# tesseract-robotics/trajopt

Measured on NVIDIA H100. Metric: converged trajectories/sec (7-DOF x 30 wp, batch 1024), higher is better.
Workload: dtype f64

## Files before the change

### trajopt_b200/csrc/kernels.h

```cpp
#pragma once
#include "device_types.cuh"

namespace tb200 {
struct EvalExtra;
struct SolveCtl;
using SolveKernelFn = void (*)(DevProblem, EvalExtra, SolveCtl);
using EvalKernelFn = void (*)(DevProblem, EvalExtra, int, const double*);
SolveKernelFn solve_kernel_for(int D, bool pair_rows, bool sing);
EvalKernelFn eval_kernel_for(int D, bool sing);
int eval_debug_prof(unsigned long long* out, int reset);
constexpr int kQpProfSlots = 32;
int qp_debug_prof(unsigned long long* out, int reset);
}
```

### trajopt_b200/csrc/qp_cta_kernel.cuh

```cuda
#pragma once
#include "device_types.cuh"
#include "joint_terms.cuh"

namespace tb200 {

#ifdef TB200_PROFILE
static __device__ unsigned long long g_prof[32];
#define PROF_T0() const long long prof_t0_ = clock64()
#define PROF_ADD(slot) do { if (q.tid == 0) atomicAdd(&g_prof[slot], (unsigned long long)(clock64() - prof_t0_)); } while (0)
#define PROF_COUNT(slot) do { if (q.tid == 0) atomicAdd(&g_prof[slot], 1ull); } while (0)
#define PROF_ADD2(slot, slot2) do { if (q.tid == 0) { const unsigned long long d_ = clock64() - prof_t0_; \
    atomicAdd(&g_prof[slot], d_); atomicAdd(&g_prof[slot2], d_); } } while (0)
#else
#define PROF_T0()
#define PROF_ADD(slot)
#define PROF_COUNT(slot)
#define PROF_ADD2(slot, slot2)
#endif
#if defined(TB200_PROFILE) && defined(TB200_PROFILE_CHECK)
#define PROF_CHK_T0() long long pc_ = clock64()
#define PROF_CHK(slot) do { const long long n_ = clock64(); if (q.tid == 0) atomicAdd(&g_prof[slot], (unsigned long long)(n_ - pc_)); pc_ = n_; } while (0)
#else
#define PROF_CHK_T0()
#define PROF_CHK(slot)
#endif

constexpr int kQpThreads = 256;
constexpr int kQpThreadsC = 256;
constexpr double kOsqpInf = 1e30;
constexpr double kMinScaling = 1e-4, kMaxScaling = 1e4;
constexpr double kVerifyTol = 1e-9;
constexpr int kVerifyRounds = 3;
constexpr double kRhoMin = 1e-6, kRhoMax = 1e6, kRhoTol = 1e-4, kRhoEqOverIneq = 1e3;
enum { QPS_UNSOLVED = 0, QPS_SOLVED = 1, QPS_SOLVED_INACC = 2, QPS_PINF = 3, QPS_PINF_INACC = 4, QPS_DINF = 5,
       QPS_DINF_INACC = 6, QPS_MAXITER = 7, QPS_NONCVX = 8 };

__device__ __forceinline__ double limit_scaling(double v) {
  v = v < kMinScaling ? 1.0 : v;
  return v > kMaxScaling ? kMaxScaling : v;
}

struct QpSmem {
  int SA, SLM, SU, beta, x, zb, yb, v1, w, qs, lbs, ubs, Dz, v2, Pb, tmp, red, colptr, colent, rints, rows, total, row_cap;
  int factor_smem, pband_smem;
  int pinv;
};

struct PinvPlan {
  int ok;
  int Ns, nS;
  int PR;
  int ZS, HO;
  int WS;
  int SS;
  int zo, wo, so;
  int total;
};
__host__ __device__ inline PinvPlan pinv_plan(int M, int nb) {
  PinvPlan pl;
  pl.Ns = M / 4;
  pl.nS = pl.Ns * nb;
  pl.PR = (M - pl.Ns) * nb;
  const int Np = M * nb, blk = nb * nb;
  pl.ok = (nb % 2 == 0) && nb <= 14 && pl.Ns <= 3 && pl.PR + 2 * pl.nS <= 256;
  pl.ZS = Np + ((4 - Np % 16) + 16) % 16;
  pl.HO = ((Np / 2 + 6) / 16) * 16 + 2;
  if (pl.HO > Np) pl.HO = Np;
  pl.WS = 2 * nb + 2;
  pl.SS = pl.nS + (pl.nS & 1);
  const int fA = (M * blk + 15) & ~15, fL = fA + 8, fU = (M * blk + 1) & ~1;
  const int zn = pl.nS * pl.ZS;
  pl.zo = 0;
  pl.wo = ((zn > fA + fL + fU ? zn : fA + fL + fU) + 15) & ~15;
  pl.so = pl.wo + ((pl.PR * pl.WS + 1) & ~1);
  pl.total = pl.so + pl.nS * pl.SS;
  return pl;
}
constexpr int kQpSmemBudget = 28800;
__host__ __device__ inline int qp_block_count(int N, int nb) { return (N + nb - 1) / nb; }
__host__ __device__ inline int qp_even(int v) { return (v + 1) & ~1; }
__host__ __device__ inline int qp_factor_doubles(int N, int nb) { return 3 * qp_even(qp_block_count(N, nb) * nb * nb); }
__host__ __device__ inline size_t qp_cta_global_doubles(int N, int nb) {
  const PinvPlan pl = pinv_plan(qp_block_count(N, nb), nb);
  return static_cast<size_t>(qp_factor_doubles(N, nb)) + static_cast<size_t>(pl.nS) * pl.ZS;
}
__host__ __device__ inline QpSmem qp_smem_layout(int N, int nb, int row_stride, int CN, int max_rows, bool factor_global) {
  const int M = qp_block_count(N, nb), Np = M * nb, blk = nb * nb;
  QpSmem s;
  int o = 0;
  s.beta = o; o += qp_even(Np);
  s.x = o;    o += qp_even(Np);
  s.zb = o;   o += qp_even(Np);
  s.yb = o;   o += qp_even(Np);
  s.v1 = o;   o += qp_even(Np);
  s.w = o;    o += qp_even(Np);
  s.qs = o;   o += qp_even(Np);
  s.lbs = o;  o += qp_even(Np);
  s.ubs = o;  o += qp_even(Np);
  s.Dz = o;   o += qp_even(Np);
  s.v2 = o;   o += qp_even(Np);
  s.tmp = o;  o += 2 * kQpThreadsC + 64 + 8;
  s.red = o;  o += 16 * 8;
  s.colptr = o; o += qp_even((Np + 2) / 2 + 1);
  const int fA = (M * blk + 15) & ~15, fL = fA + 8, fU = qp_even(M * blk);
  s.factor_smem = (!factor_global && o + fA + fL + fU <= kQpSmemBudget) ? 1 : 0;
  o = s.factor_smem ? ((o + 15) & ~15) : o;
  const int per_row2 = 2 * row_stride + CN + RI_NINTS;
  const PinvPlan pl = pinv_plan(M, nb);
  {
    const int region = qp_even(pl.total > fA + fL + fU ? pl.total : fA + fL + fU);
    const int o2 = o + region + qp_even(N * (nb + 1));
    const int cap2 = (o2 < kQpSmemBudget) ? 2 * (kQpSmemBudget - o2) / per_row2 - 1 : 0;
    s.pinv = (s.factor_smem && pl.ok && cap2 >= (max_rows < 64 ? max_rows : 64)) ? 1 : 0;
  }
  s.SA = o;   o += s.factor_smem ? fA : 0;
  s.SLM = o;  o += s.factor_smem ? fL : 0;
  s.SU = o;   o += s.factor_smem ? fU : 0;
  if (s.pinv && s.SA + pl.total > o) o = s.SA + qp_even(pl.total);
  s.pband_smem = (o + qp_even(N * (nb + 1)) <= kQpSmemBudget) ? 1 : 0;
  s.Pb = o;   o += s.pband_smem ? qp_even(N * (nb + 1)) : 0;
  int cap = (o < kQpSmemBudget) ? 2 * (kQpSmemBudget - o) / per_row2 - 1 : 0;
  cap = cap > max_rows ? max_rows : cap;
  cap = cap > 1023 ? 1023 : cap;
  cap = cap < 0 ? 0 : cap;
  s.row_cap = cap;
  s.colent = o; o += qp_even((cap * CN + 1) / 2);
  s.rints = o;  o += qp_even((cap * RI_NINTS + 1) / 2);
  s.rows = o;   o += cap * row_stride;
  s.total = o;
  return s;
}

enum RowF {
  R_C = 0, R_W,
  R_E, R_DA0, R_DA1, R_EA0, R_EA1,
  R_U0, R_U1, R_B0, R_B1, R_LO, R_UP, R_QA0, R_QA1, R_RHO,
  R_XA0, R_XA1, R_Z, R_Y, R_ZA0, R_ZA1, R_YA0, R_YA1,
  R_RA0, R_RA1, R_COEF, R_WR, R_G0, R_G1, R_DEN, R_WRR,
  R_IDEN, R_IWRR,
  R_DY, R_DYA0, R_DYA1, R_DXA0, R_DXA1,
  R_PW, R_PWA0, R_PWA1, R_PB, R_PY, R_PYA0, R_PYA1, R_PX0, R_PX1,
  R_MV,
  R_NF
};
__host__ __device__ inline int qp_row_stride(int CN) { return 3 * CN + R_NF; }

struct SmVec {
  int off;
  __device__ __forceinline__ double* ptr() const {
    extern __shared__ double sm[];
    return sm + off;
  }
  __device__ __forceinline__ double& operator[](int i) const { return ptr()[i]; }
  __device__ __forceinline__ operator double*() const { return ptr(); }
  __device__ __forceinline__ SmVec& operator=(double* p) {
    extern __shared__ double sm[];
    off = static_cast<int>(p - sm);
    return *this;
  }
};

struct QpCtx {
  int N, Np, nb, M, T, D, CN, RS, tid, nrows;
  double *SA, *SLM, *SU;
  SmVec beta, x, zb, yb, v1, w, qs, lbs, ubs, tmp, red, flag;
  int* colptr;
  SmVec Dz, v2;
  double* rows;
  double* soa;
  double* smbase;
  int rows_smem;
  int* rints;
  const int* colent;
  const double* Pband;
  const int* band_offs;
  int n_band;
  double* scratch;
  int pinv;
  PinvPlan pl;
  double* pi_g;
  double* z_stash;
  double c, cinv, rho, rho_eq, sigma, alpha;
  __device__ __forceinline__ double* R(int r) const { return rows + static_cast<size_t>(r) * RS; }
  __device__ __forceinline__ double* F(int r) const { return rows + static_cast<size_t>(r) * RS + 2 * CN; }
  __device__ __forceinline__ const int* I(int r) const { return rints + static_cast<size_t>(r) * RI_NINTS; }
};

__device__ __forceinline__ double warp_max_norm(double v) {
  v = (v != v) ? 0.0 : v;
  const unsigned hi = static_cast<unsigned>(__double2hiint(v)) & 0x7fffffffu, lo = static_cast<unsigned>(__double2loint(v));
  const unsigned mh = __reduce_max_sync(0xffffffffu, hi);
  const unsigned ml = __reduce_max_sync(0xffffffffu, hi == mh ? lo : 0u);
  return __hiloint2double(static_cast<int>(mh), static_cast<int>(ml));
}
template <int NQ, unsigned SUM_MASK>
__device__ __forceinline__ void block_reduce(const QpCtx& q, double (&vals)[NQ]) {
  static_assert(NQ <= 16, "red area too small");
  extern __shared__ double sm[];
  double* const red = sm + (q.red - q.smbase);
  const int lane = q.tid & 31, wid = q.tid >> 5;
  __syncwarp();
#pragma unroll
  for (int k = 0; k < NQ; ++k) {
    double v = vals[k];
    if ((SUM_MASK >> k) & 1u) {
#pragma unroll
      for (int off = 16; off > 0; off >>= 1) v += __shfl_xor_sync(0xffffffffu, v, off);
    } else {
      v = warp_max_norm(v);
    }
    vals[k] = v;
  }
  if (lane == 0) {
#pragma unroll
    for (int k = 0; k < NQ; ++k) red[k * 8 + wid] = vals[k];
  }
  __syncthreads();
#pragma unroll
  for (int k = 0; k < NQ; ++k) {
    if ((SUM_MASK >> k) & 1u) {
      double acc = red[k * 8];
#pragma unroll
      for (int w = 1; w < kQpThreads / 32; ++w) acc += red[k * 8 + w];
      vals[k] = acc;
    } else {
      vals[k] = warp_max_norm(red[k * 8 + (lane & 7)]);
    }
  }
  __syncthreads();
}

struct SysW {
  bool polish;
  double sig, rho_aux;
#ifdef TB200_PROFILE
  int prof_kind = 0;
#endif
};

__device__ __forceinline__ int row_var(const int* I, int k) {
  return I[RI_BASE] + min(k, I[RI_CNT] - 1) * I[RI_STRIDE];
}

template <int NB>
__device__ __forceinline__ void load_row(double (&a)[NB], const double* src) {
  const double2* s2 = reinterpret_cast<const double2*>(src);
#pragma unroll
  for (int k = 0; k < NB / 2; ++k) {
    const double2 v = s2[k];
    a[2 * k] = v.x;
    a[2 * k + 1] = v.y;
  }
}
template <int NB>
__device__ __forceinline__ void store_row(double* dst, const double (&a)[NB]) {
  double2* d2 = reinterpret_cast<double2*>(dst);
#pragma unroll
  for (int k = 0; k < NB / 2; ++k) d2[k] = make_double2(a[2 * k], a[2 * k + 1]);
}
template <int NB>
__device__ __forceinline__ void row_times_mat(double (&out)[NB], const double (&x)[NB], const double* Y) {
#pragma unroll
  for (int k = 0; k < NB; ++k) {
    double y[NB];
    load_row<NB>(y, Y + k * NB);
#pragma unroll
    for (int j = 0; j < NB; ++j) out[j] += x[k] * y[j];
  }
}
template <int NB>
__device__ __forceinline__ void row_times_matT(double (&out)[NB], const double (&x)[NB], const double* Y) {
#pragma unroll
  for (int j = 0; j < NB; ++j) {
    double y[NB];
    load_row<NB>(y, Y + j * NB);
    double a0 = 0.0, a1 = 0.0;
#pragma unroll
    for (int k = 0; k < NB; k += 2) {
      a0 += x[k] * y[k];
      a1 += x[k + 1] * y[k + 1];
    }
    out[j] += a0 + a1;
  }
}
template <int NB, bool WARP>
__device__ inline bool bcr_factor(const QpCtx& q) {
  static_assert(!WARP || NB <= 16, "a block per half warp");
  constexpr int BLK = NB * NB, G = kQpThreads / 2;
  constexpr int CH1 = WARP ? kQpThreads / 16 : kQpThreads / NB, CH2 = G / NB;
  extern __shared__ double sm[];
  double* const SA = WARP ? sm + (q.SA - q.smbase) : q.SA;
  double* const SLM = WARP ? sm + (q.SLM - q.smbase) : q.SLM;
  double* const SU = WARP ? sm + (q.SU - q.smbase) : q.SU;
  const int M = q.M, tid = q.tid;
  const int grp = tid >= G, gt = tid - (grp ? G : 0);
  int bad = 0;
  for (int l = 0; (1 << l) - 1 < M; ++l) {
    const int s = 1 << l, first = s - 1, sh = l + 1;
    const int nE = (M + s) >> sh, nS = M >> sh;
    PROF_T0();
    for (int e0 = 0; e0 < nE; e0 += CH1) {
      const int nc = (nE - e0 < CH1) ? nE - e0 : CH1;
      const int e = WARP ? tid >> 4 : tid / NB, i = WARP ? tid & 15 : tid % NB;
      const bool act = WARP ? (i < NB && e < nc) : tid < nc * NB;
      double* A = SA + (first + ((e0 + (act ? e : 0)) << sh)) * BLK + (act ? i : 0) * NB;
      double a[NB];
      load_row<NB>(a, A);
#pragma unroll
      for (int k = 0; k < NB; ++k) {
        double* prow = q.tmp + (k & 1) * (CH1 * NB) + e * NB;
// ... 322 lines not shown
  for (int k = 0; k < H; ++k) {
    a0 += xx[2 * k] * yy[k].x;
    a1 += xx[2 * k + 1] * yy[k].y;
  }
#pragma unroll
  for (int k = 0; k < H; ++k) a2 += um[k] * ww[k];
  const double dx = a0 + a1;
  return (side ? (hasr ? -dx : 0.0) : dx) - (hasl ? a2 : 0.0);
}
template <int NB>
__device__ __forceinline__ void bcr_solve_sm(const int tid, const SolveRoles& R, const double* sm_base, double* v, double* w) {
  const int wbase = tid & ~31;
  const bool side = tid & 1;
#if defined(TB200_PROFILE) && !defined(TB200_PROFILE_CHECK)
  long long pt_ = clock64();
#define PROF_LVL(slot) do { const long long n_ = clock64(); if (tid == 0) atomicAdd(&g_prof[slot], (unsigned long long)(n_ - pt_)); pt_ = n_; } while (0)
#else
#define PROF_LVL(slot)
#endif
  __syncthreads();
  PROF_LVL(4);
  if (wbase < R.f0_warps) {
    double a = bcr_fwd_task<NB>(sm_base + R.f0_mat, v + R.f0_vec);
    a = R.f0_valid ? a : 0.0;
    const double o = __shfl_xor_sync(0xffffffffu, a, 1);
    if (R.f0_store) v[R.f0_dst] -= a + o;
  }
  __syncthreads();
  PROF_LVL(14);
  for (int l = 1; l < R.n_fwd; ++l) {
    const bool mine = R.fu_level == l;
    if (__any_sync(0xffffffffu, mine)) {
      double a = bcr_fwd_task<NB>(sm_base + (mine ? R.fu_mat : 0), v + (mine ? R.fu_vec : 0));
      a = (mine && R.fu_valid) ? a : 0.0;
      const double o = __shfl_xor_sync(0xffffffffu, a, 1);
      if (mine && R.fu_store) v[R.fu_dst] -= a + o;
    }
    __syncthreads();
  }
  PROF_LVL(15);
  for (int l = R.n_lvl - 1; l >= 1; --l) {
    const bool mine = R.bu_level == l;
    if (__any_sync(0xffffffffu, mine)) {
      double acc = bcr_bwd_task<NB>(sm_base + (mine ? R.bu_X : 0), sm_base + (mine ? R.bu_Um : 0),
                                    (R.bu_yw ? w : v) + (mine ? R.bu_y : 0), w + (mine ? R.bu_wl : 0), R.bu_yw, R.bu_hasl,
                                    R.bu_hasr);
      acc = mine ? acc : 0.0;
      const double o = __shfl_xor_sync(0xffffffffu, acc, 1);
      if (mine && R.bu_store) w[R.bu_dst] = acc + o;
    }
    __syncthreads();
  }
  PROF_LVL(9);
  if (wbase < R.b0_warps) {
    const double acc = bcr_bwd_task<NB>(sm_base + R.b0_X, sm_base + R.b0_Um, (side ? w : v) + R.b0_y, w + R.b0_wl, side,
                                        R.b0_hasl, R.b0_hasr);
    const double o = __shfl_xor_sync(0xffffffffu, acc, 1);
    if (R.b0_store) w[R.b0_dst] = acc + o;
  }
  __syncthreads();
}

template <int NB>
__device__ __forceinline__ double reg_bwd_task(const double (&m)[NB + NB / 2], const double* y, const double* wl, bool side,
                                               bool hasl, bool hasr) {
  constexpr int H = NB / 2;
  double2 yy[H];
  double ww[H];
#pragma unroll
  for (int k = 0; k < H; ++k) yy[k] = lds_v2(y + 2 * k);
#pragma unroll
  for (int k = 0; k < H; ++k) ww[k] = lds_f64(wl + k);
  double a0 = 0.0, a1 = 0.0, a2 = 0.0;
#pragma unroll
  for (int k = 0; k < H; ++k) {
    a0 += m[2 * k] * yy[k].x;
    a1 += m[2 * k + 1] * yy[k].y;
  }
#pragma unroll
  for (int k = 0; k < H; ++k) a2 += m[NB + k] * ww[k];
  const double dx = a0 + a1;
  return (side ? (hasr ? -dx : 0.0) : dx) - (hasl ? a2 : 0.0);
}

template <int NB>
__device__ __forceinline__ void bcr_solve_hyb(const int tid, const SolveRoles& R, const double (&mB0)[NB + NB / 2],
                                              const double* sm_base, double* v, double* w) {
  const int wbase = tid & ~31;
  const bool side = tid & 1;
  __syncthreads();
  if (wbase < R.f0_warps) {
    double a = bcr_fwd_task<NB>(sm_base + R.f0_mat, v + R.f0_vec);
    a = R.f0_valid ? a : 0.0;
    const double o = __shfl_xor_sync(0xffffffffu, a, 1);
    if (R.f0_store) v[R.f0_dst] -= a + o;
  }
  __syncthreads();
  for (int l = 1; l < R.n_fwd; ++l) {
    const bool mine = R.fu_level == l;
    if (__any_sync(0xffffffffu, mine)) {
      double a = bcr_fwd_task<NB>(sm_base + (mine ? R.fu_mat : 0), v + (mine ? R.fu_vec : 0));
      a = (mine && R.fu_valid) ? a : 0.0;
      const double o = __shfl_xor_sync(0xffffffffu, a, 1);
      if (mine && R.fu_store) v[R.fu_dst] -= a + o;
    }
    __syncthreads();
  }
  for (int l = R.n_lvl - 1; l >= 1; --l) {
    const bool mine = R.bu_level == l;
    if (__any_sync(0xffffffffu, mine)) {
      double acc = bcr_bwd_task<NB>(sm_base + (mine ? R.bu_X : 0), sm_base + (mine ? R.bu_Um : 0),
                                    (R.bu_yw ? w : v) + (mine ? R.bu_y : 0), w + (mine ? R.bu_wl : 0), R.bu_yw, R.bu_hasl,
                                    R.bu_hasr);
      acc = mine ? acc : 0.0;
      const double o = __shfl_xor_sync(0xffffffffu, acc, 1);
      if (mine && R.bu_store) w[R.bu_dst] = acc + o;
    }
    __syncthreads();
  }
  if (wbase < R.b0_warps) {
    const double acc = reg_bwd_task<NB>(mB0, (side ? w : v) + R.b0_y, w + R.b0_wl, side, R.b0_hasl, R.b0_hasr);
    const double o = __shfl_xor_sync(0xffffffffu, acc, 1);
    if (R.b0_store) w[R.b0_dst] = acc + o;
  }
  __syncthreads();
}

template <int NB>
__device__ __forceinline__ double p_row(const QpCtx& q, const int i, const double* Dz, const double* vin) {
  constexpr int HB = NB, W = HB + 1;
  const int N = q.N, nbo = q.n_band;
  const double* const Pb = q.Pband;
  const int* const offs = q.band_offs;
  double s = 0.0;
  for (int t0 = 0; t0 < nbo; t0 += 4) {
    double v[4];
#pragma unroll
    for (int u = 0; u < 4; ++u) {
      const int k = (t0 + u < nbo) ? offs[t0 + u] : -1;
      v[u] = (k >= 0 && k <= i) ? (Pb[i * W + k] * Dz[i - k]) * vin[i - k] : 0.0;
    }
    s += v[0]; s += v[1]; s += v[2]; s += v[3];
  }
  for (int t0 = 0; t0 < nbo; t0 += 4) {
    double v[4];
#pragma unroll
    for (int u = 0; u < 4; ++u) {
      const int k = (t0 + u < nbo) ? offs[t0 + u] : -1;
      v[u] = (k >= 1 && i + k < N) ? (Pb[(i + k) * W + k] * Dz[i + k]) * vin[i + k] : 0.0;
    }
    s += v[0]; s += v[1]; s += v[2]; s += v[3];
  }
  return s * (q.c * Dz[i]);
}
template <int NB>
__device__ __forceinline__ void p_matvec(const QpCtx& q, const double* in, double* out) {
  extern __shared__ double sm[];
  const int N = q.N, Np = q.Np;
  const double* const Dz = sm + (q.Dz - q.smbase);
  const double* const vin = sm + (in - q.smbase);
  double* const vout = sm + (out - q.smbase);
  for (int i = q.tid; i < Np; i += kQpThreads) vout[i] = (i < N) ? p_row<NB>(q, i, Dz, vin) : 0.0;
  __syncthreads();
}

__device__ __forceinline__ void info_row_terms(const double* F, const double ax, double (&m)[14]) {
  const double einv = 1.0 / F[R_E];
  m[0] = fmax(m[0], fabs(einv * (ax - F[R_Z])));
  m[1] = fmax(m[1], fabs(einv * F[R_Z]));
  m[2] = fmax(m[2], fabs(einv * ax));
  m[7] = fmax(m[7], fabs(ax - F[R_Z]));
  m[8] = fmax(m[8], fabs(F[R_Z]));
  m[9] = fmax(m[9], fabs(ax));
#pragma unroll
  for (int k = 0; k < 2; ++k) {
    const double u = F[R_U0 + k], bb = F[R_B0 + k], qa = F[R_QA0 + k];
    const double xa = F[R_XA0 + k], za = F[R_ZA0 + k], ya = F[R_YA0 + k];
    const double iea = 1.0 / F[R_EA0 + k], ida = 1.0 / F[R_DA0 + k];
    const double axb = bb * xa;
    m[0] = fmax(m[0], fabs(iea * (axb - za)));
    m[1] = fmax(m[1], fabs(iea * za));
    m[2] = fmax(m[2], fabs(iea * axb));
    m[7] = fmax(m[7], fabs(axb - za));
    m[8] = fmax(m[8], fabs(za));
    m[9] = fmax(m[9], fabs(axb));
    const double aty = u * F[R_Y] + bb * ya;
    m[3] = fmax(m[3], fabs(ida * (qa + aty)));
    m[4] = fmax(m[4], fabs(ida * aty));
    m[5] = fmax(m[5], fabs(ida * qa));
    m[10] = fmax(m[10], fabs(qa + aty));
    m[11] = fmax(m[11], fabs(aty));
    m[12] = fmax(m[12], fabs(qa));
  }
}
__device__ __forceinline__ void info_var_terms(const double dz, const double beta, const double x, const double zb,
                                               const double aty, const double px, const double qv, double (&m)[14]) {
  const double ax = beta * x;
  const double einv = dz / beta, dinv = 1.0 / dz;
  m[0] = fmax(m[0], fabs(einv * (ax - zb)));
  m[1] = fmax(m[1], fabs(einv * zb));
  m[2] = fmax(m[2], fabs(einv * ax));
  m[7] = fmax(m[7], fabs(ax - zb));
  m[8] = fmax(m[8], fabs(zb));
  m[9] = fmax(m[9], fabs(ax));
  const double d = qv + px + aty;
  m[3] = fmax(m[3], fabs(dinv * d));
  m[4] = fmax(m[4], fabs(dinv * aty));
  m[5] = fmax(m[5], fabs(dinv * qv));
  m[6] = fmax(m[6], fabs(dinv * px));
  m[10] = fmax(m[10], fabs(d));
  m[11] = fmax(m[11], fabs(aty));
  m[12] = fmax(m[12], fabs(qv));
  m[13] = fmax(m[13], fabs(px));
}
__device__ __forceinline__ double pinf_row_terms(const double* F, const int naux, double (&a)[3]) {
  double d = F[R_DY];
  d = (naux == AUX_HINGE) ? fmax(d, 0.0) : d;
  a[0] = fmax(a[0], fabs(F[R_E] * d));
  a[1] += F[R_UP] * fmax(d, 0.0) + F[R_LO] * fmin(d, 0.0);
#pragma unroll
  for (int k = 0; k < 2; ++k) {
    const double da = fmin(F[R_DYA0 + k], 0.0);
    a[0] = fmax(a[0], fabs(F[R_EA0 + k] * da));
    a[2] = fmax(a[2], fabs((F[R_U0 + k] * d + F[R_B0 + k] * da) / F[R_DA0 + k]));
  }
  return d;
}
__device__ __forceinline__ void pinf_var_terms(const double ratio, const double ub, const double lb, const double d,
                                               double (&a)[3]) {
  a[0] = fmax(a[0], fabs(ratio * d));
  a[1] += ub * fmax(d, 0.0) + lb * fmin(d, 0.0);
}
__device__ __forceinline__ void dinf_row_terms(const double* F, double (&a)[2]) {
#pragma unroll
  for (int k = 0; k < 2; ++k) {
    a[0] = fmax(a[0], fabs(F[R_DA0 + k] * F[R_DXA0 + k]));
    a[1] += F[R_QA0 + k] * F[R_DXA0 + k];
  }
}
__device__ __forceinline__ unsigned long long guess_mix(unsigned long long v) {
  v += 0x9e3779b97f4a7c15ull;
  v = (v ^ (v >> 30)) * 0xbf58476d1ce4e5b9ull;
  v = (v ^ (v >> 27)) * 0x94d049bb133111ebull;
  return v ^ (v >> 31);
}
__device__ __forceinline__ unsigned long long guess_row_hash(const double* F, const int* I, const int r, const int nrows,
                                                             const int N) {
  unsigned long long h = 0ull;
  const unsigned long long mc = static_cast<unsigned long long>(nrows);
  if (F[R_Z] - F[R_LO] < -F[R_Y]) h += guess_mix(2ull * r);
  else if (F[R_UP] - F[R_Z] < F[R_Y]) h += guess_mix(2ull * r + 1ull);
  for (int k = 0; k < I[RI_AUX]; ++k) {
    const unsigned long long idx = mc + N + I[RI_PAD] + k;
    if (F[R_ZA0 + k] - 0.0 < -F[R_YA0 + k]) h += guess_mix(2ull * idx);
    else if (kOsqpInf * F[R_EA0 + k] - F[R_ZA0 + k] < F[R_YA0 + k]) h += guess_mix(2ull * idx + 1ull);
  }
  return h;
}
__device__ __forceinline__ unsigned long long guess_var_hash(const double zb, const double yb, const double lb,
                                                             const double ub, const int i, const int nrows) {
  const unsigned long long idx = static_cast<unsigned long long>(nrows) + i;
  if (zb - lb < -yb) return guess_mix(2ull * idx);
  if (ub - zb < yb) return guess_mix(2ull * idx + 1ull);
  return 0ull;
}
enum ChkQ { CHK_PA0 = 14, CHK_PA1, CHK_PA2, CHK_DA0, CHK_DA1, kChkHash };
constexpr unsigned kChkSumMask = (1u << CHK_PA1) | (1u << CHK_DA1);

__device__ inline void rows_prepare_weights(const QpCtx& q, const SysW& w) {
  for (int r = q.tid; r < q.nrows; r += kQpThreads) {
    double* F = q.F(r);
    const int naux = q.I(r)[RI_AUX];
    const double Wr = w.polish ? fabs(F[R_PW]) : ((F[R_RHO] != 0.0) ? q.rho_eq : q.rho);
    const double wa0 = w.polish ? fabs(F[R_PWA0]) : w.rho_aux;
    const double wa1 = w.polish ? fabs(F[R_PWA1]) : w.rho_aux;
    const double g0 = (naux >= 1) ? w.sig + wa0 * F[R_B0] * F[R_B0] : 1.0;
    const double g1 = (naux == 2) ? w.sig + wa1 * F[R_B1] * F[R_B1] : 1.0;
    const double den = g0 * g1 + Wr * (F[R_U0] * F[R_U0] * g1 + F[R_U1] * F[R_U1] * g0);
    F[R_WRR] = Wr;
    F[R_G0] = g0;
    F[R_G1] = g1;
    F[R_DEN] = den;
    F[R_IDEN] = 1.0 / den;
    F[R_IWRR] = (Wr != 0.0) ? 1.0 / Wr : 0.0;
    F[R_WR] = Wr * g0 * g1 / den;
  }
  __syncthreads();
}
__device__ __forceinline__ double xbound_weight(const QpCtx& q, const SysW& w, int j) {
  const double adm = (q.ubs[j] - q.lbs[j] < kRhoTol) ? q.rho_eq : q.rho;
  return w.polish ? fabs(q.zb[j]) : adm;
}

__device__ __forceinline__ double pivot_rcp(const double x) {
  double r;
  asm("rcp.approx.ftz.f64 %0, %1;" : "=d"(r) : "d"(x));
  double e = fma(-x, r, 1.0);
  r = fma(r, e, r);
  e = fma(-x, r, 1.0);
  r = fma(r, e, r);
  e = fma(-x, r, 1.0);
  return fma(r, e, r);
}
template <int QN>
__device__ __forceinline__ bool gj_rows(double (&a)[QN], double diag, const bool active, const int mat, const int row,
                                        const int n, const int n_max, double* tmp, const int nmat, const int bar) {
  constexpr int BS = QN + 2;
  double* const csv = tmp + 2 * nmat * BS + mat * QN;
  bool bad = false;
  double pv_mine = pivot_rcp(diag), my_cs = 1.0, rs = 1.0, inv_rs = 1.0;
#pragma unroll 1
  for (int k = 0; k < n_max; ++k) {
    double* buf = tmp + ((k & 1) * nmat + mat) * BS;
    const bool piv = active && row == k;
    if (piv) {
      bad |= !(diag > 0.0);
#pragma unroll
      for (int j = 0; j < QN; j += 2) *reinterpret_cast<double2*>(buf + j) = make_double2(a[j], a[j + 1]);
      buf[k] = 0.0;
      buf[QN] = pv_mine;
      my_cs = -pv_mine;
      csv[k] = my_cs;
      rs = pv_mine;
      inv_rs = diag;
      diag = pv_mine;
    }
    asm volatile("bar.sync %0, 64;" ::"r"(bar) : "memory");
    if (active && k < n && !piv) {
      const double tr = buf[row];
      const bool ahead = row > k;
      const double f = ahead ? tr : -tr * my_cs;
      const double g = f * buf[QN];
      diag = ahead ? diag - g * f : diag + g * f;
      const double gs = g * inv_rs;
#pragma unroll
      for (int j = 0; j < QN; j += 2) {
        const double2 t = *reinterpret_cast<const double2*>(buf + j);
        a[j] -= gs * t.x;
        a[j + 1] -= gs * t.y;
      }
      if (ahead) pv_mine = pivot_rcp(diag);
    }
  }
  if (active) {
#pragma unroll
    for (int j = 0; j < QN; ++j) a[j] = (j == row) ? diag : ((j < n) ? a[j] * (rs * csv[j]) : 0.0);
  }
  return bad;
}

template <int NB>
__device__ inline bool pinv_factor(const QpCtx& q) {
  constexpr int QN = 3 * NB, blk = NB * NB;
  static_assert(QN % 2 == 0, "pivot rows move as double2");
  static_assert(QN <= 64, "a partition on two warps");
  extern __shared__ double sm[];
  const int tid = q.tid, M = q.M, Np = q.Np;
  const int PR = q.pl.PR, nS = q.pl.nS, Ns = q.pl.Ns, ZS = q.pl.ZS, WS = q.pl.WS, SS = q.pl.SS;
  double* const fbase = sm + (q.SA - q.smbase);
  const double* const SA = fbase;
  const double* const SLM = sm + (q.SLM - q.smbase);
  double* const Z = fbase + q.pl.zo;
  double* const W = fbase + q.pl.wo;
  double* const S = fbase + q.pl.so;
  double* const tmp = q.tmp.ptr();
  const int nparts = (M + 3) / 4;
  bool bad = false;
#ifdef TB200_PROFILE
  long long pf_ = clock64();
#define PROF_PF(slot) do { const long long n_ = clock64(); if (tid == 0) atomicAdd(&g_prof[slot], (unsigned long long)(n_ - pf_)); pf_ = n_; } while (0)
#else
#define PROF_PF(slot)
#endif
  {
    const int p = tid >> 6, lr = tid & 63, pr = p * QN + lr;
    const bool part = p < nparts;
    const int npb = !part ? 0 : (M - 4 * p) < 3 ? (M - 4 * p) : 3;
    const bool prow = lr < npb * NB;
    const int kb = lr / NB, r = lr % NB, gb = 4 * p + kb;
    double a[QN];
#pragma unroll
    for (int j = 0; j < QN; ++j) {
      const int cb = j / NB, c = j % NB;
      double v = 0.0;
      if (prow && cb < npb) {
        if (cb == kb) v = SA[gb * blk + r * NB + c];
        else if (cb == kb - 1) v = SLM[gb * blk + r * NB + c];
        else if (cb == kb + 1) v = SLM[(gb + 1) * blk + c * NB + r];
      }
      a[j] = v;
    }
    PROF_PF(0);
    const double dg = prow ? SA[gb * blk + r * NB + r] : 1.0;
    if (part) bad |= gj_rows<QN>(a, dg, prow, p, lr, npb * NB, (M < 3 ? M : 3) * NB, tmp, nparts, 1 + p);
    PROF_PF(4);
    if (prow) {
#pragma unroll
      for (int j = 0; j < QN; ++j) q.pi_g[j * PR + pr] = a[j];
      const bool has_l = p > 0, has_r = 4 * p + 3 < M;
#pragma unroll 2
      for (int j = 0; j < NB; ++j) {
        double wl = 0.0, wr = 0.0;
        if (has_l) {
#pragma unroll
          for (int c = 0; c < NB; ++c) wl += a[c] * SLM[(4 * p) * blk + c * NB + j];
        }
        if (has_r) {
#pragma unroll
          for (int c = 0; c < NB; ++c) wr += a[2 * NB + c] * SLM[(4 * p + 3) * blk + j * NB + c];
        }
        W[pr * WS + j] = wl;
        W[pr * WS + NB + j] = wr;
      }
    }
  }
  __syncthreads();
  for (int e = tid; e < nS * nS; e += kQpThreads) {
    const int ra = e / nS, ca = e % nS, sa = ra / NB, i = ra % NB, sb = ca / NB, j = ca % NB;
    double v = 0.0;
    if (sa == sb || sb == sa + 1 || sb == sa - 1) {
      const bool use_l = sb <= sa, use_r = sb >= sa && 4 * sa + 4 < M;
      const double* cl = SLM + (4 * sa + 3) * blk + i * NB;
      const double* wl = W + (sa * QN + 2 * NB) * WS + (sb == sa ? NB : 0) + j;
      const double* cr = SLM + (4 * sa + 4) * blk + i;
      const double* wr = W + ((sa + 1) * QN) * WS + (sb == sa ? 0 : NB) + j;
      double s0 = 0.0, s1 = 0.0, s2 = 0.0, s3 = 0.0;
      if (use_l) {
#pragma unroll
        for (int rr = 0; rr < NB; rr += 2) {
          s0 += cl[rr] * wl[rr * WS];
          s1 += cl[rr + 1] * wl[(rr + 1) * WS];
        }
      }
      if (use_r) {
#pragma unroll
        for (int rr = 0; rr < NB; rr += 2) {
          s2 += cr[rr * NB] * wr[rr * WS];
          s3 += cr[(rr + 1) * NB] * wr[(rr + 1) * WS];
        }
      }
      v = ((sa == sb) ? SA[(4 * sa + 3) * blk + i * NB + j] : 0.0) - ((s0 + s1) + (s2 + s3));
    }
    S[ra * SS + ca] = v;
  }
  __syncthreads();
  PROF_PF(14);
  {
    const bool srow = tid < nS;
    double a[QN];
#pragma unroll
    for (int j = 0; j < QN; ++j) a[j] = (srow && j < nS) ? S[tid * SS + j] : 0.0;
    const double dg = srow ? S[tid * SS + tid] : 1.0;
    if (tid < 64) bad |= gj_rows<QN>(a, dg, srow, 0, tid, nS, nS, tmp, 1, 1);
    if (srow) {
#pragma unroll
      for (int j = 0; j < QN; ++j)
        if (j < nS) S[tid * SS + j] = a[j];
    }
  }
  __syncthreads();
  PROF_PF(15);
  if (tid < Np) {
    const int col = tid, cb = col / NB, c = col % NB, p = cb / 4;
    if (cb % 4 == 3) {
      for (int sr = 0; sr < nS; ++sr) Z[sr * ZS + col] = S[sr * SS + p * NB + c];
    } else {
      const bool has_l = p > 0, has_r = 4 * p + 3 < M;
      const double* wrow = W + (p * QN + (cb % 4) * NB + c) * WS;
      double wv[2 * NB];
#pragma unroll
      for (int t = 0; t < 2 * NB; ++t) wv[t] = wrow[t];
      const double* sl = S + (has_l ? (p - 1) * NB : 0);
      const double* sr_ = S + (has_r ? p * NB : 0);
#pragma unroll 2
      for (int sr = 0; sr < nS; ++sr) {
        double s0 = 0.0, s1 = 0.0, s2 = 0.0, s3 = 0.0;
#pragma unroll
        for (int t = 0; t < NB; t += 2) {
          s0 += sl[sr * SS + t] * wv[t];
          s1 += sl[sr * SS + t + 1] * wv[t + 1];
          s2 += sr_[sr * SS + t] * wv[NB + t];
          s3 += sr_[sr * SS + t + 1] * wv[NB + t + 1];
        }
        Z[sr * ZS + col] = -((s0 + s1) + (s2 + s3));
      }
    }
  }
  (void)Ns;
  const bool ok = !__syncthreads_or(bad ? 1 : 0);
  PROF_PF(9);
  return ok;
}

template <int NB, bool PINV, bool WARP>
__device__ __noinline__ bool assemble_factor(const QpCtx& q, const SysW& w) {
  PROF_T0();
  rows_prepare_weights(q, w);
  constexpr int nb = NB, blk = NB * NB;
  extern __shared__ double sm[];
  constexpr bool SMEM = PINV || WARP;
  double* const SA = SMEM ? sm + (q.SA - q.smbase) : q.SA;
  double* const SLM = SMEM ? sm + (q.SLM - q.smbase) : q.SLM;
  const int N = q.N, HB = 2 * q.D, PW = HB + 1, CN = q.CN;
  for (int t = q.tid; t < q.M * blk; t += kQpThreads) {
    SA[t] = 0.0;
    SLM[t] = 0.0;
  }
  __syncthreads();
  for (int i = q.tid; i < q.Np; i += kQpThreads) {
    const int p = i / nb, r = i % nb;
    double* Arow = SA + static_cast<size_t>(p) * blk + r * nb;
    double* Lrow = SLM + static_cast<size_t>(p) * blk + r * nb;
    if (i >= N) {
      Arow[r] = 1.0;
      continue;
    }
    auto add = [&](int k, double val) {
      if (k <= r) Arow[r - k] = __dadd_rn(Arow[r - k], val);
      else Lrow[nb + r - k] = __dadd_rn(Lrow[nb + r - k], val);
    };
    for (int t = 0; t < q.n_band; ++t) {
      const int k = q.band_offs[t];
      if (k <= i) add(k, q.c * q.Dz[i] * q.Pband[i * PW + k] * q.Dz[i - k]);
    }
    add(0, w.sig + xbound_weight(q, w, i) * q.beta[i] * q.beta[i]);
    for (int e = q.colptr[i]; e < q.colptr[i + 1]; ++e) {
      const int ent = q.colent[e], rw = ent >> 5, k = ent & 31;
      const double* R = q.R(rw);
      const double wr = R[2 * CN + R_WR];
      if (wr == 0.0) continue;
      const int stride = q.I(rw)[RI_STRIDE];
      const double* as = R + CN;
      const double ai = wr * as[k];
      for (int k2 = 0; k2 <= k; ++k2) add((k - k2) * stride, ai * as[k2]);
    }
  }
  __syncthreads();
  for (int t = q.tid; t < q.M * blk; t += kQpThreads) {
    const int p = t / blk, i = (t % blk) / nb, j = t % nb;
    if (j > i) SA[static_cast<size_t>(p) * blk + i * nb + j] = SA[static_cast<size_t>(p) * blk + j * nb + i];
  }
  __syncthreads();
#ifdef TB200_PROFILE
  const int pk = w.polish ? 2 : w.prof_kind;
  if (pk == 1) PROF_COUNT(31);
#endif
  PROF_ADD2(10, 24 + 2 * pk);
  bool ok;
  {
    PROF_T0();
    if constexpr (PINV) ok = pinv_factor<NB>(q);
    else ok = bcr_factor<NB, WARP>(q);
    PROF_ADD2(11, 25 + 2 * pk);
  }
  return ok;
}

struct QpPlan {
  bool use_reg, use_pinv, fuse, fast_polish;
};
__host__ __device__ inline QpPlan qp_plan(bool regok, int pinv, int rows_smem, int M, int nb, bool fast_passes) {
  QpPlan pl;
  pl.use_reg = regok && solve_roles_fit(M, nb);
  pl.use_pinv = regok && pinv && rows_smem;
  pl.fuse = pl.use_pinv && fast_passes;
  pl.fast_polish = pl.use_pinv && fast_passes && M * nb <= kQpThreads && solve_roles_fit(M, nb);
  return pl;
}
enum QpPath {
  QPP_BLOCK_PINV = 1 << 0,
  QPP_BLOCK_FAST = 1 << 1,
  QPP_BLOCK_GENERIC = 1 << 2,
  QPP_BLOCK_SOA = 1 << 3,
  QPP_FACTOR_GLOBAL = 1 << 4,
  QPP_BAND_GLOBAL = 1 << 5,
  QPP_ROWS_GLOBAL = 1 << 6,
  QPP_FUSED_CHECK = 1 << 7,
  QPP_POLISH_FAST = 1 << 8,
  QPP_POLISH_GENERIC = 1 << 9
};
__host__ __device__ inline int qp_plan_block(const QpPlan& pl, int rows_smem) {
  if (pl.use_pinv) return QPP_BLOCK_PINV;
  if (!rows_smem) return QPP_BLOCK_SOA;
  return pl.use_reg ? QPP_BLOCK_FAST : QPP_BLOCK_GENERIC;
}

struct QpOut {
  int status, iters, polish;
  double rho;
  double pri_res, dua_res, pol_pri, pol_dua, c;
  int pol_factor_ok, rho_updates, rounds;
};

template <int CN, class Base>
__device__ __forceinline__ void scatter_columns(const QpCtx& q, Base base) {
  for (int i = q.tid; i < q.Np; i += kQpThreads) {
    double s = 0.0;
    if (i < q.N) {
      s = base(i);
      for (int e = q.colptr[i]; e < q.colptr[i + 1]; ++e) {
        const int ent = q.colent[e], r = ent >> 5, k = ent & 31;
        const double* R = q.R(r);
        s += R[CN + k] * R[2 * CN + R_COEF];
      }
    }
    q.v1[i] = s;
  }
  __syncthreads();
}
template <int CN>
__device__ __forceinline__ double row_dot(const QpCtx& q, const double* R, const int* I, const double* v) {
  double z = 0.0;
  const int base = I[RI_BASE], stride = I[RI_STRIDE], last = I[RI_CNT] - 1;
#pragma unroll
  for (int k = 0; k < CN; ++k) z += R[CN + k] * v[base + min(k, last) * stride];
  return z;
}
__device__ __forceinline__ void row_backsub(const double* F, double zeta, double& a0, double& a1) {
  const double Wr = F[R_WRR], ra0 = F[R_RA0], ra1 = F[R_RA1], u0 = F[R_U0], u1 = F[R_U1];
  const double iden = F[R_IDEN];
  a0 = (F[R_G1] * (ra0 - Wr * u0 * zeta) + Wr * u1 * (u1 * ra0 - u0 * ra1)) * iden;
  a1 = (F[R_G0] * (ra1 - Wr * u1 * zeta) + Wr * u0 * (u0 * ra1 - u1 * ra0)) * iden;
}
__device__ __forceinline__ double row_reduce_coef(const double* F, double ra0, double ra1, double zcoef) {
  return zcoef - F[R_WRR] * (F[R_U0] * ra0 * F[R_G1] + F[R_U1] * ra1 * F[R_G0]) * F[R_IDEN];
}
template <int CNc>
__device__ __forceinline__ void admm_row_entry(const double* R, double* F, const double& sigma, const double& rho_aux) {
  const double s = F[R_WRR] * F[R_Z] - F[R_Y];
  const double ra0 = sigma * F[R_XA0] - F[R_QA0] + F[R_U0] * s + F[R_B0] * (rho_aux * F[R_ZA0] - F[R_YA0]);
  const double ra1 = sigma * F[R_XA1] - F[R_QA1] + F[R_U1] * s + F[R_B1] * (rho_aux * F[R_ZA1] - F[R_YA1]);
  F[R_RA0] = ra0;
  F[R_RA1] = ra1;
  const double cf = row_reduce_coef(F, ra0, ra1, s);
  F[R_COEF] = cf;
#pragma unroll
  for (int k = 0; k < CNc; ++k) F[R_NF + k] = R[CNc + k] * cf;
}
template <int CNc>
__device__ __forceinline__ void admm_row_update(const double* R, double* F, const int* I, const double* w,
                                                const double& sigma, const double& alpha, const double& oma,
                                                const double& rho_aux, const double& inv_rho_aux) {
  double zeta = 0.0;
  {
    const int base = I[RI_BASE], stride = I[RI_STRIDE], last = I[RI_CNT] - 1;
#pragma unroll
    for (int k = 0; k < CNc; ++k) zeta += R[CNc + k] * w[base + min(k, last) * stride];
  }
  double a0, a1;
  row_backsub(F, zeta, a0, a1);
  const double zt = zeta + F[R_U0] * a0 + F[R_U1] * a1;
  const double Wr = F[R_WRR];
  const double zr = alpha * zt + oma * F[R_Z];
  double zn = zr + F[R_Y] * F[R_IWRR];
  zn = fmin(fmax(zn, F[R_LO]), F[R_UP]);
  const double dy = Wr * (zr - zn);
  const double yn = F[R_Y] + dy;
  F[R_Z] = zn;
  F[R_Y] = yn;
  F[R_DY] = dy;
  const double s = Wr * zn - yn;
  double ra[2];
#pragma unroll
  for (int k = 0; k < 2; ++k) {
    const double at = k ? a1 : a0, bb = F[R_B0 + k];
    const double xo = F[R_XA0 + k];
    const double xn = alpha * at + oma * xo;
    const double zra = alpha * (bb * at) + oma * F[R_ZA0 + k];
    double z2 = zra + F[R_YA0 + k] * inv_rho_aux;
    z2 = fmin(fmax(z2, 0.0), kOsqpInf * F[R_EA0 + k]);
    const double dya = rho_aux * (zra - z2);
    const double yan = F[R_YA0 + k] + dya;
    F[R_XA0 + k] = xn;
    F[R_DXA0 + k] = xn - xo;
    F[R_ZA0 + k] = z2;
    F[R_YA0 + k] = yan;
    F[R_DYA0 + k] = dya;
    ra[k] = sigma * xn - F[R_QA0 + k] + F[R_U0 + k] * s + bb * (rho_aux * z2 - yan);
  }
  F[R_RA0] = ra[0];
  F[R_RA1] = ra[1];
  const double cf = row_reduce_coef(F, ra[0], ra[1], s);
  F[R_COEF] = cf;
#pragma unroll
  for (int k = 0; k < CNc; ++k) F[R_NF + k] = R[CNc + k] * cf;
}

template <int NB, int PAIR>
__device__ __noinline__ void admm_block(const QpCtx& q, const double rho_aux, const int n_iter, const int keep_last) {
  constexpr int CNc = PAIR ? ((NB > 3) ? NB : 3) : ((NB / 2 > 3) ? NB / 2 : 3);
  const int N = q.N, tid = q.tid;
  double* const dxs = q.scratch;
  double* const dyb = q.scratch + q.Np;
  const bool one_var = q.Np <= kQpThreads;
  const int my_e0 = (one_var && tid < N) ? q.colptr[tid] : 0, my_e1 = (one_var && tid < N) ? q.colptr[tid + 1] : 0;
  {
    PROF_T0();
    for (int r = kQpThreads - 1 - tid; r < q.nrows; r += kQpThreads)
      admm_row_entry<CNc>(q.R(r), q.F(r), q.sigma, rho_aux);
    __syncthreads();
    PROF_ADD(0);
  }
  const double inv_rho_aux = 1.0 / rho_aux;
  const double inv_rho = 1.0 / q.rho, inv_rho_eq = 1.0 / q.rho_eq;
  for (int it = 0; it < n_iter; ++it) {
    const bool keep_steps = keep_last && it == n_iter - 1;
    {
      PROF_T0();
      if (one_var) {
        const int i = tid;
        double s = 0.0;
        if (i < N) {
          const double rb = (q.ubs[i] - q.lbs[i] < kRhoTol) ? q.rho_eq : q.rho;
          s = q.sigma * q.x[i] - q.qs[i] + q.beta[i] * (rb * q.zb[i] - q.yb[i]);
          for (int e = my_e0; e < my_e1; ++e) {
            const int ent = q.colent[e];
            s += q.rows[static_cast<size_t>(ent >> 5) * q.RS + (2 * CNc + R_NF) + (ent & 31)];
          }
        }
        if (i < q.Np) q.v1[i] = s;
      } else {
        for (int i = tid; i < q.Np; i += kQpThreads) {
          double s = 0.0;
          if (i < N) {
            const double rb = (q.ubs[i] - q.lbs[i] < kRhoTol) ? q.rho_eq : q.rho;
            s = q.sigma * q.x[i] - q.qs[i] + q.beta[i] * (rb * q.zb[i] - q.yb[i]);
            for (int e = q.colptr[i]; e < q.colptr[i + 1]; ++e) {
              const int ent = q.colent[e];
              s += q.rows[static_cast<size_t>(ent >> 5) * q.RS + (2 * CNc + R_NF) + (ent & 31)];
            }
          }
          q.v1[i] = s;
        }
      }
      PROF_ADD(1);
    }
    {
      PROF_T0();
      bcr_solve<NB>(q, q.v1, q.w);
      PROF_ADD(2);
    }
    PROF_T0();
    for (int r = kQpThreads - 1 - tid; r < q.nrows; r += kQpThreads)
      admm_row_update<CNc>(q.R(r), q.F(r), q.I(r), q.w, q.sigma, q.alpha, 1.0 - q.alpha, rho_aux, inv_rho_aux);
    for (int i = tid; i < N; i += kQpThreads) {
      const double beta = q.beta[i];
      const double lb = q.lbs[i], ub = q.ubs[i];
      const bool beq = ub - lb < kRhoTol;
      const double rb = beq ? q.rho_eq : q.rho, irb = beq ? inv_rho_eq : inv_rho;
      const double xt = q.w[i];
      const double xn = q.alpha * xt + (1.0 - q.alpha) * q.x[i];
      const double zr = q.alpha * (beta * xt) + (1.0 - q.alpha) * q.zb[i];
      double zn = zr + q.yb[i] * irb;
      zn = fmin(fmax(zn, lb), ub);
      const double dy = rb * (zr - zn);
      if (keep_steps) {
        dxs[i] = xn - q.x[i];
        dyb[i] = dy;
      }
      q.x[i] = xn;
      q.zb[i] = zn;
      q.yb[i] += dy;
    }
    __syncthreads();
    PROF_ADD(3);
  }
}

template <int NB, int PAIR>
__device__ __noinline__ void admm_block_fast(const QpCtx& q, const double rho_aux_in, const int n_iter, const int keep_last) {
  constexpr int CNc = PAIR ? ((NB > 3) ? NB : 3) : ((NB / 2 > 3) ? NB / 2 : 3);
  constexpr int kPre = 8;
  extern __shared__ double sm[];
  const int tid = q.tid, N = q.N, Np = q.Np, nrows = q.nrows, RS = q.RS;
  const double sigma = q.sigma, alpha = q.alpha, oma = 1.0 - q.alpha, rho = q.rho, rho_eq = q.rho_eq, rho_aux = rho_aux_in;
  const double inv_rho_aux = 1.0 / rho_aux, inv_rho = 1.0 / rho, inv_rho_eq = 1.0 / rho_eq;
  double* const v1 = sm + (q.v1 - q.smbase);
  double* const w = sm + (q.w - q.smbase);
  double* const rows = sm + (q.rows - q.smbase);
  const int* const rints = reinterpret_cast<const int*>(sm + (reinterpret_cast<const double*>(q.rints) - q.smbase));
  const int* const colent = reinterpret_cast<const int*>(sm + (reinterpret_cast<const double*>(q.colent) - q.smbase));
  double* const dxs = q.scratch;
  double* const dyb = q.scratch + Np;
  const SolveRoles roles = solve_roles<NB>(q);
  double mB0[NB + NB / 2];
  load_bwd_row<NB>(q, 0, tid, mB0);
  const bool has_var = tid < N;
  const int vi = has_var ? tid : 0;
  const double v_beta = q.beta[vi], v_lb = q.lbs[vi], v_ub = q.ubs[vi], v_qs = q.qs[vi];
  const bool v_eq = v_ub - v_lb < kRhoTol;
  const double v_rb = v_eq ? rho_eq : rho, v_irb = v_eq ? inv_rho_eq : inv_rho;
  double v_x = q.x[vi], v_z = q.zb[vi], v_y = q.yb[vi];
  const int e0 = has_var ? q.colptr[vi] : 0, e1 = has_var ? q.colptr[vi + 1] : 0;
// ... 1696 lines not shown
```

Baseline: 1473.

## Pipeline next pivot row publication in Gauss-Jordan and vectorize pinv shared loads

```diff
diff --git a/trajopt_b200/csrc/kernels.h b/trajopt_b200/csrc/kernels.h
--- a/trajopt_b200/csrc/kernels.h
+++ b/trajopt_b200/csrc/kernels.h
@@ -9,6 +9,6 @@
 SolveKernelFn solve_kernel_for(int D, bool pair_rows, bool sing);
 EvalKernelFn eval_kernel_for(int D, bool sing);
 int eval_debug_prof(unsigned long long* out, int reset);
-constexpr int kQpProfSlots = 32;
+constexpr int kQpProfSlots = 64;
 int qp_debug_prof(unsigned long long* out, int reset);
 }
diff --git a/trajopt_b200/csrc/qp_cta_kernel.cuh b/trajopt_b200/csrc/qp_cta_kernel.cuh
--- a/trajopt_b200/csrc/qp_cta_kernel.cuh
+++ b/trajopt_b200/csrc/qp_cta_kernel.cuh
@@ -5,7 +5,7 @@
 namespace tb200 {
 
 #ifdef TB200_PROFILE
-static __device__ unsigned long long g_prof[32];
+static __device__ unsigned long long g_prof[64];
 #define PROF_T0() const long long prof_t0_ = clock64()
 #define PROF_ADD(slot) do { if (q.tid == 0) atomicAdd(&g_prof[slot], (unsigned long long)(clock64() - prof_t0_)); } while (0)
 #define PROF_COUNT(slot) do { if (q.tid == 0) atomicAdd(&g_prof[slot], 1ull); } while (0)
@@ -934,50 +934,115 @@
   e = fma(-x, r, 1.0);
   return fma(r, e, r);
 }
+#if defined(TB200_PROFILE) && defined(TB200_PROFILE_PF)
+#define TB200_PF 1
+#endif
+#if defined(TB200_PROFILE) && defined(TB200_PROFILE_PF_HASH)
+#define TB200_PF_HASH 1
+#endif
+#if defined(TB200_PF) || defined(TB200_PF_HASH)
+__device__ __forceinline__ unsigned long long pf_mix(const double v, const unsigned idx) {
+  unsigned long long z = static_cast<unsigned long long>(__double_as_longlong(v)) ^ (idx * 0x9E3779B97F4A7C15ull);
+  z = (z ^ (z >> 30)) * 0xBF58476D1CE4E5B9ull;
+  z = (z ^ (z >> 27)) * 0x94D049BB133111EBull;
+  return z ^ (z >> 31);
+}
+__device__ __forceinline__ void pf_warp_add(const int slot, unsigned long long v) {
+#pragma unroll
+  for (int o = 16; o > 0; o >>= 1) v += __shfl_xor_sync(0xffffffffu, v, o);
+  if ((threadIdx.x & 31) == 0) atomicAdd(&g_prof[slot], v);
+}
+#endif
 template <int QN>
 __device__ __forceinline__ bool gj_rows(double (&a)[QN], double diag, const bool active, const int mat, const int row,
-                                        const int n, const int n_max, double* tmp, const int nmat, const int bar) {
+                                        const int n, const int n_max, double* tmp, const int nmat, const int bar,
+                                        const int pslot) {
   constexpr int BS = QN + 2;
   double* const csv = tmp + 2 * nmat * BS + mat * QN;
   bool bad = false;
-  double pv_mine = pivot_rcp(diag), my_cs = 1.0, rs = 1.0, inv_rs = 1.0;
+  double my_cs = 1.0, rs = 1.0, inv_rs = 1.0;
+  auto become_pivot = [&](double* pub, const int k, const double pv) {
+    pub[k] = 0.0;
+    pub[QN] = pv;
+    bad |= !(diag > 0.0);
+    my_cs = -pv;
+    csv[k] = my_cs;
+    rs = pv;
+    inv_rs = diag;
+    diag = pv;
+  };
+#ifdef TB200_PF
+  long long pf_upd = 0, pf_wait = 0;
+  const long long pf_in = clock64();
+#endif
+  if (active && row == 0) {
+    double* const pub = tmp + mat * BS;
+#pragma unroll
+    for (int j = 0; j < QN; j += 2) *reinterpret_cast<double2*>(pub + j) = make_double2(a[j], a[j + 1]);
+    become_pivot(pub, 0, pivot_rcp(diag));
+  }
 #pragma unroll 1
   for (int k = 0; k < n_max; ++k) {
-    double* buf = tmp + ((k & 1) * nmat + mat) * BS;
-    const bool piv = active && row == k;
-    if (piv) {
-      bad |= !(diag > 0.0);
-#pragma unroll
-      for (int j = 0; j < QN; j += 2) *reinterpret_cast<double2*>(buf + j) = make_double2(a[j], a[j + 1]);
-      buf[k] = 0.0;
-      buf[QN] = pv_mine;
-      my_cs = -pv_mine;
-      csv[k] = my_cs;
-      rs = pv_mine;
-      inv_rs = diag;
-      diag = pv_mine;
-    }
+    const double* const buf = tmp + ((k & 1) * nmat + mat) * BS;
+    double* const pub = tmp + ((~k & 1) * nmat + mat) * BS;
+#ifdef TB200_PF
+    const long long pf_t1 = clock64();
+#endif
     asm volatile("bar.sync %0, 64;" ::"r"(bar) : "memory");
-    if (active && k < n && !piv) {
+#ifdef TB200_PF
+    const long long pf_t2 = clock64();
+    if (active && row == k) pf_wait = pf_t2 - pf_t1;
+#endif
+    if (active && k < n && row != k) {
       const double tr = buf[row];
       const bool ahead = row > k;
+      const bool nxt = row == k + 1;
       const double f = ahead ? tr : -tr * my_cs;
       const double g = f * buf[QN];
       diag = ahead ? diag - g * f : diag + g * f;
       const double gs = g * inv_rs;
+      double pv = 0.0;
+      if (nxt) pv = pivot_rcp(diag);
+      double2 t[QN / 2];
+#pragma unroll
+      for (int j = 0; j < QN; j += 2) t[j / 2] = *reinterpret_cast<const double2*>(buf + j);
 #pragma unroll
       for (int j = 0; j < QN; j += 2) {
-        const double2 t = *reinterpret_cast<const double2*>(buf + j);
-        a[j] -= gs * t.x;
-        a[j + 1] -= gs * t.y;
-      }
-      if (ahead) pv_mine = pivot_rcp(diag);
-    }
-  }
+        a[j] -= gs * t[j / 2].x;
+        a[j + 1] -= gs * t[j / 2].y;
+        if (nxt) *reinterpret_cast<double2*>(pub + j) = make_double2(a[j], a[j + 1]);
+      }
+      if (nxt) become_pivot(pub, k + 1, pv);
+#ifdef TB200_PF
+      if (nxt) pf_upd = clock64() - pf_t2 + (pv != pv);
+#endif
+    }
+  }
+#ifdef TB200_PF
+  const long long pf_loop = clock64();
+  {
+    const bool c = active && row >= 1;
+    pf_warp_add(pslot + 1, c ? pf_wait : 0);
+    pf_warp_add(pslot + 2, c ? pf_upd : 0);
+    pf_warp_add(pslot + 4, c ? 1 : 0);
+  }
+#else
+  (void)pslot;
+#endif
   if (active) {
 #pragma unroll
-    for (int j = 0; j < QN; ++j) a[j] = (j == row) ? diag : ((j < n) ? a[j] * (rs * csv[j]) : 0.0);
-  }
+    for (int j = 0; j < QN; ++j) {
+      const double s = a[j] * (rs * csv[j]);
+      a[j] = (j == row) ? diag : ((j < n) ? s : 0.0);
+    }
+  }
+#ifdef TB200_PF
+  if (threadIdx.x == 0) {
+    const int lb = (pslot == 41) ? 57 : 60;
+    atomicAdd(&g_prof[lb], (unsigned long long)(pf_loop - pf_in));
+    atomicAdd(&g_prof[lb + 1], (unsigned long long)(clock64() + (a[QN - 1] != a[QN - 1]) - pf_loop));
+  }
+#endif
   return bad;
 }
 
@@ -998,11 +1063,23 @@
   double* const tmp = q.tmp.ptr();
   const int nparts = (M + 3) / 4;
   bool bad = false;
-#ifdef TB200_PROFILE
+#ifdef TB200_PF
   long long pf_ = clock64();
 #define PROF_PF(slot) do { const long long n_ = clock64(); if (tid == 0) atomicAdd(&g_prof[slot], (unsigned long long)(n_ - pf_)); pf_ = n_; } while (0)
+  if (tid == 0) {
+    atomicAdd(&g_prof[32], 1ull);
+    atomicAdd(&g_prof[39], (unsigned long long)((M < 3 ? M : 3) * NB));
+    atomicAdd(&g_prof[40], (unsigned long long)nS);
+  }
 #else
 #define PROF_PF(slot)
+#endif
+#ifdef TB200_PF_HASH
+#define PF_HASH(h, v, idx) h += pf_mix(v, idx)
+  unsigned long long h_pi = 0, h_w = 0, h_s = 0, h_z = 0;
+  if (tid == 0) atomicAdd(&g_prof[56], 1ull);
+#else
+#define PF_HASH(h, v, idx)
 #endif
   {
     const int p = tid >> 6, lr = tid & 63, pr = p * QN + lr;
@@ -1014,37 +1091,67 @@
 #pragma unroll
     for (int j = 0; j < QN; ++j) {
       const int cb = j / NB, c = j % NB;
-      double v = 0.0;
-      if (prow && cb < npb) {
-        if (cb == kb) v = SA[gb * blk + r * NB + c];
-        else if (cb == kb - 1) v = SLM[gb * blk + r * NB + c];
-        else if (cb == kb + 1) v = SLM[(gb + 1) * blk + c * NB + r];
-      }
-      a[j] = v;
-    }
-    PROF_PF(0);
+      if constexpr (NB > 4) {
+        const bool nz = prow && cb < npb && (cb == kb || cb == kb - 1 || cb == kb + 1);
+        const int off = (cb == kb + 1) ? (gb + 1) * blk + c * NB + r : gb * blk + r * NB + c;
+        const double v = (cb == kb ? SA : SLM)[nz ? off : 0];
+        a[j] = nz ? v : 0.0;
+      } else {
+        double v = 0.0;
+        if (prow && cb < npb) {
+          if (cb == kb) v = SA[gb * blk + r * NB + c];
+          else if (cb == kb - 1) v = SLM[gb * blk + r * NB + c];
+          else if (cb == kb + 1) v = SLM[(gb + 1) * blk + c * NB + r];
+        }
+        a[j] = v;
+      }
+    }
+    PROF_PF(33);
     const double dg = prow ? SA[gb * blk + r * NB + r] : 1.0;
-    if (part) bad |= gj_rows<QN>(a, dg, prow, p, lr, npb * NB, (M < 3 ? M : 3) * NB, tmp, nparts, 1 + p);
-    PROF_PF(4);
+    if (part) bad |= gj_rows<QN>(a, dg, prow, p, lr, npb * NB, (M < 3 ? M : 3) * NB, tmp, nparts, 1 + p, 41);
+    PROF_PF(34);
     if (prow) {
 #pragma unroll
-      for (int j = 0; j < QN; ++j) q.pi_g[j * PR + pr] = a[j];
+      for (int j = 0; j < QN; ++j) {
+        q.pi_g[j * PR + pr] = a[j];
+        PF_HASH(h_pi, a[j], j * PR + pr);
+      }
       const bool has_l = p > 0, has_r = 4 * p + 3 < M;
-#pragma unroll 2
-      for (int j = 0; j < NB; ++j) {
-        double wl = 0.0, wr = 0.0;
-        if (has_l) {
-#pragma unroll
-          for (int c = 0; c < NB; ++c) wl += a[c] * SLM[(4 * p) * blk + c * NB + j];
+      double w[2 * NB];
+#pragma unroll
+      for (int j = 0; j < 2 * NB; ++j) w[j] = 0.0;
+      if (has_l) {
+        const double* const cl = SLM + (4 * p) * blk;
+#pragma unroll
+        for (int c = 0; c < NB; ++c) {
+#pragma unroll
+          for (int j = 0; j < NB; j += 2) {
+            const double2 t = *reinterpret_cast<const double2*>(cl + c * NB + j);
+            w[j] += a[c] * t.x;
+            w[j + 1] += a[c] * t.y;
+          }
         }
-        if (has_r) {
-#pragma unroll
-          for (int c = 0; c < NB; ++c) wr += a[2 * NB + c] * SLM[(4 * p + 3) * blk + j * NB + c];
+      }
+      if (has_r) {
+        const double* const cr = SLM + (4 * p + 3) * blk;
+#pragma unroll
+        for (int c = 0; c < NB; c += 2) {
+#pragma unroll
+          for (int j = 0; j < NB; ++j) {
+            const double2 t = *reinterpret_cast<const double2*>(cr + j * NB + c);
+            w[NB + j] += a[2 * NB + c] * t.x;
+            w[NB + j] += a[2 * NB + c + 1] * t.y;
+          }
         }
-        W[pr * WS + j] = wl;
-        W[pr * WS + NB + j] = wr;
-      }
-    }
+      }
+#pragma unroll
+      for (int j = 0; j < 2 * NB; j += 2) {
+        *reinterpret_cast<double2*>(W + pr * WS + j) = make_double2(w[j], w[j + 1]);
+        PF_HASH(h_w, w[j], pr * WS + j);
+        PF_HASH(h_w, w[j + 1], pr * WS + j + 1);
+      }
+    }
+    PROF_PF(35);
   }
   __syncthreads();
   for (int e = tid; e < nS * nS; e += kQpThreads) {
@@ -1076,26 +1183,35 @@
     S[ra * SS + ca] = v;
   }
   __syncthreads();
-  PROF_PF(14);
+  PROF_PF(36);
   {
     const bool srow = tid < nS;
     double a[QN];
 #pragma unroll
-    for (int j = 0; j < QN; ++j) a[j] = (srow && j < nS) ? S[tid * SS + j] : 0.0;
+    for (int j = 0; j < QN; ++j) {
+      const double v = S[(srow ? tid : 0) * SS + (j < nS ? j : 0)];
+      a[j] = (srow && j < nS) ? v : 0.0;
+    }
     const double dg = srow ? S[tid * SS + tid] : 1.0;
-    if (tid < 64) bad |= gj_rows<QN>(a, dg, srow, 0, tid, nS, nS, tmp, 1, 1);
+    if (tid < 64) bad |= gj_rows<QN>(a, dg, srow, 0, tid, nS, nS, tmp, 1, 1, 46);
     if (srow) {
 #pragma unroll
       for (int j = 0; j < QN; ++j)
-        if (j < nS) S[tid * SS + j] = a[j];
-    }
-  }
-  __syncthreads();
-  PROF_PF(15);
+        if (j < nS) {
+          S[tid * SS + j] = a[j];
+          PF_HASH(h_s, a[j], tid * SS + j);
+        }
+    }
+  }
+  __syncthreads();
+  PROF_PF(37);
   if (tid < Np) {
     const int col = tid, cb = col / NB, c = col % NB, p = cb / 4;
     if (cb % 4 == 3) {
-      for (int sr = 0; sr < nS; ++sr) Z[sr * ZS + col] = S[sr * SS + p * NB + c];
+      for (int sr = 0; sr < nS; ++sr) {
+        Z[sr * ZS + col] = S[sr * SS + p * NB + c];
+        PF_HASH(h_z, S[sr * SS + p * NB + c], sr * ZS + col);
+      }
     } else {
       const bool has_l = p > 0, has_r = 4 * p + 3 < M;
       const double* wrow = W + (p * QN + (cb % 4) * NB + c) * WS;
@@ -1104,23 +1220,33 @@
       for (int t = 0; t < 2 * NB; ++t) wv[t] = wrow[t];
       const double* sl = S + (has_l ? (p - 1) * NB : 0);
       const double* sr_ = S + (has_r ? p * NB : 0);
-#pragma unroll 2
+#pragma unroll 4
       for (int sr = 0; sr < nS; ++sr) {
         double s0 = 0.0, s1 = 0.0, s2 = 0.0, s3 = 0.0;
 #pragma unroll
         for (int t = 0; t < NB; t += 2) {
-          s0 += sl[sr * SS + t] * wv[t];
-          s1 += sl[sr * SS + t + 1] * wv[t + 1];
-          s2 += sr_[sr * SS + t] * wv[NB + t];
-          s3 += sr_[sr * SS + t + 1] * wv[NB + t + 1];
+          const double2 l = *reinterpret_cast<const double2*>(sl + sr * SS + t);
+          const double2 r = *reinterpret_cast<const double2*>(sr_ + sr * SS + t);
+          s0 += l.x * wv[t];
+          s1 += l.y * wv[t + 1];
+          s2 += r.x * wv[NB + t];
+          s3 += r.y * wv[NB + t + 1];
         }
         Z[sr * ZS + col] = -((s0 + s1) + (s2 + s3));
+        PF_HASH(h_z, -((s0 + s1) + (s2 + s3)), sr * ZS + col);
       }
     }
   }
   (void)Ns;
   const bool ok = !__syncthreads_or(bad ? 1 : 0);
-  PROF_PF(9);
+  PROF_PF(38);
+#ifdef TB200_PF_HASH
+  pf_warp_add(52, h_pi);
+  pf_warp_add(53, h_w);
+  pf_warp_add(54, h_s);
+  pf_warp_add(55, h_z);
+#endif
+#undef PF_HASH
   return ok;
 }
 
```

Measured after the change: 1488 (median of 6 runs). No clear change (+1.0%).
